# jshilong/GPT4RoI

Hardware: NVIDIA B200
Metric: samples_per_sec_prefill_336px_8roi_128tok_7b (higher is better)
Workload: dtype bf16

## Files before the change

gpt4roi_b200/csrc/attention_tcgen05.cu:

```cuda
#include <stdlib.h>

#include "common.cuh"
#include "ptx.cuh"
#include "act_type.cuh"

namespace G4R_NS {

constexpr int kFaBM = 128;
constexpr int kFaThreads = 256;
constexpr int kAtomBytes = 128 * 128;

struct FaParams {
  __nv_bfloat16* out;
  long long ldo, bso;
  int L, H;
  float scale;
  const int* seqlens;
  float* lse;
};

__device__ __forceinline__ void tmem_st_32x32b_x32(uint32_t taddr, const uint32_t (&r)[32]) {
  asm volatile(
      "tcgen05.st.sync.aligned.32x32b.x32.b32 [%0], "
      "{%1, %2, %3, %4, %5, %6, %7, %8, %9, %10, %11, %12, %13, %14, %15, %16, "
      "%17, %18, %19, %20, %21, %22, %23, %24, %25, %26, %27, %28, %29, %30, %31, %32};"
      ::"r"(taddr), "r"(r[0]), "r"(r[1]), "r"(r[2]), "r"(r[3]), "r"(r[4]), "r"(r[5]), "r"(r[6]), "r"(r[7]),
      "r"(r[8]), "r"(r[9]), "r"(r[10]), "r"(r[11]), "r"(r[12]), "r"(r[13]), "r"(r[14]), "r"(r[15]), "r"(r[16]),
      "r"(r[17]), "r"(r[18]), "r"(r[19]), "r"(r[20]), "r"(r[21]), "r"(r[22]), "r"(r[23]), "r"(r[24]),
      "r"(r[25]), "r"(r[26]), "r"(r[27]), "r"(r[28]), "r"(r[29]), "r"(r[30]), "r"(r[31])
      : "memory");
}
__device__ __forceinline__ void tmem_st_wait() { asm volatile("tcgen05.wait::st.sync.aligned;" ::: "memory"); }

using ptx::make_smem_desc_mn_sw128;

template <int D, int BN, bool CAUSAL>
__global__ void __launch_bounds__(kFaThreads, (BN == 64 ? 2 : 1))
fa_fwd_tcgen05(const __grid_constant__ CUtensorMap tm_q, const __grid_constant__ CUtensorMap tm_k,
               const __grid_constant__ CUtensorMap tm_v, const __grid_constant__ FaParams p) {
  constexpr int kFaBN = BN;
  constexpr int ATOMS = D / 64;
  constexpr int Q_BYTES = ATOMS * kAtomBytes;
  constexpr int KV_ATOM = BN * 128;
  constexpr int TILE_BYTES = ATOMS * KV_ATOM;
  constexpr int P_BYTES = (BN / 64) * kAtomBytes;
  constexpr int TMEM_COLS = (2 * BN + D) <= 256 ? 256 : 512;
  extern __shared__ __align__(1024) uint8_t smem[];
  uint8_t* sQ = smem;
  uint8_t* sK = sQ + Q_BYTES;
  uint8_t* sV = sK + 2 * TILE_BYTES;
  uint8_t* sP = sV + 2 * TILE_BYTES;
// ... 1 lines not shown
  uint64_t* q_full = bars;
  uint64_t* k_full = bars + 1;
  uint64_t* k_empty = bars + 3;
  uint64_t* v_full = bars + 5;
  uint64_t* v_empty = bars + 7;
  uint64_t* s_full = bars + 9;
  uint64_t* s_free = bars + 11;
  uint64_t* p_full = bars + 13;
  uint64_t* pv_done = bars + 14;
  uint32_t* tmem_slot = reinterpret_cast<uint32_t*>(bars + 15);

  const int warp = threadIdx.x >> 5, lane = threadIdx.x & 31;
  const int qb = CAUSAL ? (int)(gridDim.x - 1 - blockIdx.x) : (int)blockIdx.x, h = blockIdx.y, b = blockIdx.z;
  const int q0 = qb * kFaBM;
  const int row_base = b * p.L;
  const int Lk = p.seqlens ? min(max(p.seqlens[b], 1), p.L) : p.L;
  const int nblk = CAUSAL ? min((Lk + kFaBN - 1) / kFaBN, (q0 + kFaBM + kFaBN - 1) / kFaBN) : (Lk + kFaBN - 1) / kFaBN;

  if (warp == 0 && lane == 0) {
    ptx::prefetch_tensormap(&tm_q);
    ptx::prefetch_tensormap(&tm_k);
    ptx::prefetch_tensormap(&tm_v);
  }
  if (warp == 1 && lane == 0) {
    ptx::mbar_init(q_full, 1);
    for (int i = 0; i < 2; i++) {
      ptx::mbar_init(&k_full[i], 1);
      ptx::mbar_init(&k_empty[i], 1);
      ptx::mbar_init(&v_full[i], 1);
      ptx::mbar_init(&v_empty[i], 1);
      ptx::mbar_init(&s_full[i], 1);
      ptx::mbar_init(&s_free[i], 128);
    }
    ptx::mbar_init(p_full, 128);
    ptx::mbar_init(pv_done, 1);
    ptx::fence_barrier_init();
  }
  if (warp == 2) ptx::tmem_alloc(tmem_slot, TMEM_COLS);
  ptx::tcgen05_before_thread_sync();
  __syncthreads();
  ptx::tcgen05_after_thread_sync();
  const uint32_t tmem_base = *tmem_slot;
  const uint32_t tmem_o = tmem_base + 2 * kFaBN;

  if (warp == 0) {
    if (lane == 0) {
      ptx::mbar_arrive_expect_tx(q_full, Q_BYTES);
      for (int a = 0; a < ATOMS; a++)
        ptx::tma_load_2d(sQ + a * kAtomBytes, &tm_q, q_full, h * D + a * 64, row_base + q0);
      for (int j = 0; j < nblk; j++) {
        const int st = j & 1;
        const uint32_t ph = (j >> 1) & 1;
        ptx::mbar_wait(&k_empty[st], ph ^ 1);
        ptx::mbar_arrive_expect_tx(&k_full[st], TILE_BYTES);
        for (int a = 0; a < ATOMS; a++)
          ptx::tma_load_2d(sK + st * TILE_BYTES + a * KV_ATOM, &tm_k, &k_full[st], h * D + a * 64,
                           row_base + j * kFaBN);
        ptx::mbar_wait(&v_empty[st], ph ^ 1);
// ... 54 lines not shown
    constexpr float kTau = 8.0f;
    float m_used = -INFINITY, l_run = 0.f;
    for (int j = 0; j < nblk; j++) {
      const int sb = j & 1;
      ptx::mbar_wait(&s_full[sb], (j >> 1) & 1);
      ptx::tcgen05_after_thread_sync();
      const uint32_t ts = tmem_base + sb * kFaBN + lane_off;
      const int key0 = j * kFaBN;
      const bool need_mask = (key0 + kFaBN > Lk) || (CAUSAL && key0 + kFaBN - 1 > q0);
      uint32_t sv[kFaBN / 32][32];
#pragma unroll
      for (int cc = 0; cc < kFaBN / 32; cc++) ptx::tmem_ld_32x32b_x32(ts + cc * 32, sv[cc]);
      ptx::tmem_ld_wait();
      ptx::tcgen05_before_thread_sync();
      ptx::mbar_arrive(&s_free[sb]);
      float mx = -INFINITY;
#pragma unroll
      for (int cc = 0; cc < kFaBN / 32; cc++) {
#pragma unroll
        for (int i = 0; i < 32; i++) {
          float sc = __uint_as_float(sv[cc][i]);
          if (need_mask) {
            const int key = key0 + cc * 32 + i;
            if (key >= Lk || (CAUSAL && key > qrow)) sc = -INFINITY;
            sv[cc][i] = __float_as_uint(sc);
          }
          mx = fmaxf(mx, sc);
        }
      }
      const float m_new = fmaxf(m_used, mx);
      const bool grow = (m_new - m_used) * c > kTau;
      float alpha = 1.f;
      if (grow) {
        alpha = exp2f((m_used - m_new) * c);
        m_used = m_new;
      }
      const float mc = (m_used == -INFINITY ? 0.f : m_used) * c;
      uint32_t pk[kFaBN / 2];
      float lsum = 0.f;
#pragma unroll
      for (int cc = 0; cc < kFaBN / 32; cc++) {
#pragma unroll
        for (int i = 0; i < 16; i++) {
          const float p0 = exp2f(fmaf(__uint_as_float(sv[cc][2 * i]), c, -mc));
          const float p1 = exp2f(fmaf(__uint_as_float(sv[cc][2 * i + 1]), c, -mc));
          lsum += p0 + p1;
          __nv_bfloat162 hh = __floats2bfloat162_rn(p0, p1);
          pk[cc * 16 + i] = *reinterpret_cast<uint32_t*>(&hh);
        }
      }
      l_run = l_run * alpha + lsum;
      if (j > 0) {
        ptx::mbar_wait(pv_done, (j - 1) & 1);
        ptx::tcgen05_after_thread_sync();
        if (__any_sync(0xffffffffu, grow)) {
#pragma unroll 1
          for (int cc = 0; cc < D / 32; cc++) {
            uint32_t v[32];
            ptx::tmem_ld_32x32b_x32(tmem_o + lane_off + cc * 32, v);
            ptx::tmem_ld_wait();
#pragma unroll
            for (int i = 0; i < 32; i++) v[i] = __float_as_uint(__uint_as_float(v[i]) * alpha);
            tmem_st_32x32b_x32(tmem_o + lane_off + cc * 32, v);
// ... 69 lines not shown
  }
  cuuint64_t dims[2] = {(cuuint64_t)cols, (cuuint64_t)rows};
  cuuint64_t str[1] = {(cuuint64_t)ld * 2};
  cuuint32_t box[2] = {64, (cuuint32_t)box_rows};
  cuuint32_t estr[2] = {1, 1};
  CUresult r = enc(m, CU_TENSOR_MAP_DATA_TYPE_BFLOAT16, 2, const_cast<void*>(base), dims, str, box, estr,
                   CU_TENSOR_MAP_INTERLEAVE_NONE, CU_TENSOR_MAP_SWIZZLE_128B, CU_TENSOR_MAP_L2_PROMOTION_L2_256B,
                   CU_TENSOR_MAP_FLOAT_OOB_FILL_NONE);
  if (r != CUDA_SUCCESS) {
    set_error("attention: cuTensorMapEncodeTiled failed (CUresult %d)", (int)r);
    return G4R_ECUDA;
  }
  return G4R_OK;
}

template <int D, int BN, bool CAUSAL>
static int launch_fa(const CUtensorMap& tq, const CUtensorMap& tk, const CUtensorMap& tv, const FaParams& p, int B,
                     cudaStream_t st) {
  constexpr int smem = (D / 64) * kAtomBytes + 4 * (D / 64) * BN * 128 + (BN / 64) * kAtomBytes + 256;
  static bool set = false;
  auto kern = fa_fwd_tcgen05<D, BN, CAUSAL>;
  if (!set) {
    G4R_CUDA(cudaFuncSetAttribute(kern, cudaFuncAttributeMaxDynamicSharedMemorySize, smem));
    set = true;
  }
  dim3 grid((p.L + kFaBM - 1) / kFaBM, p.H, B);
  kern<<<grid, kFaThreads, smem, st>>>(tq, tk, tv, p);
  G4R_LAUNCH_CHECK("fa_fwd_tcgen05");
  return G4R_OK;
}

}

using namespace G4R_NS;

static int attention_tc_impl(const void* q, const void* k, const void* v, void* out, long long ld,
                             long long bs, long long ldo, long long bso, int B, int H, int L,
                             int head_dim, int causal, float scale, const int* seqlens, float* lse, void* stream) {
  G4R_REQUIRE(q && k && v && out && B > 0 && H > 0 && L > 0, "attention_tc: bad arguments");
  G4R_REQUIRE(head_dim == 64 || head_dim == 128, "attention_tc: head_dim %d (64 or 128)", head_dim);
  G4R_REQUIRE(bs == (long long)L * ld, "attention_tc: q/k/v must be one packed [B*L, width] buffer (bs == L*ld)");
  G4R_REQUIRE(ld % 8 == 0 && ldo % 8 == 0 && bso % 8 == 0, "attention_tc: strides must keep 16-byte alignment");
  G4R_REQUIRE((((uintptr_t)q | (uintptr_t)k | (uintptr_t)v | (uintptr_t)out) & 15) == 0, "attention_tc: misaligned pointers");
  CUtensorMap tq, tk, tv;
  const long long cols = (long long)H * head_dim, rows = (long long)B * L;
  int rc;
  static int bn = 0;
  if (!bn) {
    const char* e = getenv("G4R_ATTN_BN");
    bn = (e && atoi(e) == 128) ? 128 : 64;
  }
  if ((rc = make_tmap_rows(&tq, q, cols, rows, ld, 128))) return rc;
  if ((rc = make_tmap_rows(&tk, k, cols, rows, ld, bn))) return rc;
  if ((rc = make_tmap_rows(&tv, v, cols, rows, ld, bn))) return rc;
  FaParams p{(__nv_bfloat16*)out, ldo, bso, L, H, scale, seqlens, lse};
  cudaStream_t st = (cudaStream_t)stream;
#define G4R_FA(DD, BB) (causal ? launch_fa<DD, BB, true>(tq, tk, tv, p, B, st) : launch_fa<DD, BB, false>(tq, tk, tv, p, B, st))
  if (head_dim == 64) return bn == 128 ? G4R_FA(64, 128) : G4R_FA(64, 64);
  return bn == 128 ? G4R_FA(128, 128) : G4R_FA(128, 64);
#undef G4R_FA
}

extern "C" int g4r_attention_tc_bf16(const void* q, const void* k, const void* v, void* out, long long ld,
                                     long long bs, long long ldo, long long bso, int B, int H, int L,
                                     int head_dim, int causal, float scale, const int* seqlens, void* stream) {
  return attention_tc_impl(q, k, v, out, ld, bs, ldo, bso, B, H, L, head_dim, causal, scale, seqlens, nullptr, stream);
}

#if G4R_BF16_ONLY
extern "C" int g4r_attention_tc_lse_bf16(const void* q, const void* k, const void* v, void* out, long long ld,
                                         long long bs, long long ldo, long long bso, int B, int H, int L,
                                         int head_dim, int causal, float scale, float* lse, void* stream) {
  G4R_REQUIRE(lse, "attention_tc_lse: lse is NULL");
  return attention_tc_impl(q, k, v, out, ld, bs, ldo, bso, B, H, L, head_dim, causal, scale, nullptr, lse, stream);
}
// ... 2 lines not shown
```

gpt4roi_b200/csrc/common.cuh:

```cuda
#pragma once
#include <cuda_bf16.h>
#include <cuda_fp16.h>
#include <cuda_runtime.h>
#include <stdarg.h>
#include <stdint.h>
#include <stdio.h>

#include "../../include/gpt4roi_b200.h"

namespace g4r {

void set_error(const char* fmt, ...);
int cuda_fail(cudaError_t e, const char* what);

#define G4R_REQUIRE(cond, ...)        \
  do {                                \
    if (!(cond)) {                    \
      g4r::set_error(__VA_ARGS__);    \
      return G4R_EINVAL;              \
    }                                 \
  } while (0)

#define G4R_CUDA(call)                                        \
  do {                                                        \
// ... 27 lines not shown
  if (mode == 2) pdl_release();
  pdl_wait();
  if (mode != 2) pdl_release();
}

template <typename... KArgs, typename... Args>
static inline cudaError_t launch_pdl(void (*kern)(KArgs...), dim3 grid, dim3 block, size_t smem, cudaStream_t st,
                                     dim3 cluster, Args... args) {
  cudaLaunchConfig_t cfg = {};
  cfg.gridDim = grid;
  cfg.blockDim = block;
  cfg.dynamicSmemBytes = smem;
  cfg.stream = st;
  cudaLaunchAttribute attr[2];
  int n = 0;
  attr[n].id = cudaLaunchAttributeClusterDimension;
  attr[n].val.clusterDim.x = cluster.x; attr[n].val.clusterDim.y = cluster.y; attr[n].val.clusterDim.z = cluster.z;
  n++;
  if (pdl_mode() != 0) {
    attr[n].id = cudaLaunchAttributeProgrammaticStreamSerialization;
    attr[n].val.programmaticStreamSerializationAllowed = 1;
    n++;
  }
  cfg.attrs = attr;
  cfg.numAttrs = n;
  return cudaLaunchKernelEx(&cfg, kern, static_cast<KArgs>(args)...);
}

template <typename T> __device__ __forceinline__ float to_f32(T v);
template <> __device__ __forceinline__ float to_f32<float>(float v) { return v; }
template <> __device__ __forceinline__ float to_f32<__half>(__half v) { return __half2float(v); }
template <> __device__ __forceinline__ float to_f32<__nv_bfloat16>(__nv_bfloat16 v) { return __bfloat162float(v); }

// ... 39 lines not shown
```

gpt4roi_b200/csrc/elementwise.cu:

```cuda
#include "common.cuh"
#include "act_type.cuh"

namespace G4R_NS {

__device__ __forceinline__ float warp_sum(float v) {
#pragma unroll
  for (int o = 16; o > 0; o >>= 1) v += __shfl_xor_sync(0xffffffffu, v, o);
  return v;
}

__device__ __forceinline__ void unpack8(const uint4& raw, float (&f)[8]) {
  const __nv_bfloat162* h = reinterpret_cast<const __nv_bfloat162*>(&raw);
#pragma unroll
  for (int i = 0; i < 4; i++) {
    const float2 t = __bfloat1622float2(h[i]);
    f[2 * i] = t.x;
    f[2 * i + 1] = t.y;
  }
}
__device__ __forceinline__ uint4 pack8(const float (&f)[8]) {
  uint4 raw;
  __nv_bfloat162* h = reinterpret_cast<__nv_bfloat162*>(&raw);
#pragma unroll
  for (int i = 0; i < 4; i++) h[i] = __floats2bfloat162_rn(f[2 * i], f[2 * i + 1]);
// ... 9 lines not shown
}
template <typename T> __device__ __forceinline__ void store8(T* p, const float (&f)[8]);
template <> __device__ __forceinline__ void store8<__nv_bfloat16>(__nv_bfloat16* p, const float (&f)[8]) {
  *reinterpret_cast<uint4*>(p) = pack8(f);
}
template <> __device__ __forceinline__ void store8<float>(float* p, const float (&f)[8]) {
  reinterpret_cast<float4*>(p)[0] = make_float4(f[0], f[1], f[2], f[3]);
  reinterpret_cast<float4*>(p)[1] = make_float4(f[4], f[5], f[6], f[7]);
}
__device__ __forceinline__ float bf16_round(float x) { return __bfloat162float(__float2bfloat16_rn(x)); }

template <bool RMS, int PER_LANE, typename TI = __nv_bfloat16, typename TO = __nv_bfloat16>
__global__ void __launch_bounds__(256, (sizeof(TI) == 2 && PER_LANE >= 16 ? 2 : 1))
norm_rows_bf16(const TI* __restrict__ x, long long ldx, const __nv_bfloat16* __restrict__ w,
               const __nv_bfloat16* __restrict__ b, TO* __restrict__ out, long long ldo, int M,
               int D, float eps) {
  const int row = blockIdx.x * (blockDim.x >> 5) + (threadIdx.x >> 5);
  if (row >= M) return;
  const int lane = threadIdx.x & 31;
  const int nvec = D >> 3;
  const TI* xr = x + (long long)row * ldx;
  constexpr bool PACKED = sizeof(TI) == 2;
  uint4 raw[PACKED ? PER_LANE : 1];
  float v[PACKED ? 1 : PER_LANE][8];
  float sum = 0.f, sumsq = 0.f;
#pragma unroll
  for (int i = 0; i < PER_LANE; i++) {
    const int vi = lane + (i << 5);
    float t[8];
    if (vi < nvec) {
      if constexpr (PACKED) { raw[i] = *reinterpret_cast<const uint4*>(xr + vi * 8); unpack8(raw[i], t); }
// ... 144 lines not shown
    const int per = (D / 8 + 255) / 256;
#define G4R_NORM_ROW_CASE(PR)                                                                              \
  G4R_CUDA(launch_pdl(norm_row_cta_bf16<RMS, PR>, dim3(M), dim3(256), 0, st, dim3(1, 1, 1),                \
                      (const __nv_bfloat16*)x, ldx, (const __nv_bfloat16*)w, (const __nv_bfloat16*)b,     \
                      (__nv_bfloat16*)out, ldo, D, eps, pdl_mode()))
    if (per <= 1) G4R_NORM_ROW_CASE(1);
    else if (per <= 2) G4R_NORM_ROW_CASE(2);
    else G4R_NORM_ROW_CASE(4);
#undef G4R_NORM_ROW_CASE
    G4R_LAUNCH_CHECK(RMS ? "rmsnorm" : "layernorm");
    return G4R_OK;
  }
  const int per_lane = (D / 8 + 31) / 32;
  const dim3 grid((M + 7) / 8);
#define G4R_NORM_CASE(PL)                                                                              \
  norm_rows_bf16<RMS, PL><<<grid, 256, 0, st>>>((const __nv_bfloat16*)x, ldx, (const __nv_bfloat16*)w,   \
                                                 (const __nv_bfloat16*)b, (__nv_bfloat16*)out, ldo, M, D, eps)
  if (per_lane <= 1) G4R_NORM_CASE(1);
  else if (per_lane <= 2) G4R_NORM_CASE(2);
  else if (per_lane <= 4) G4R_NORM_CASE(4);
  else if (per_lane <= 8) G4R_NORM_CASE(8);
  else if (per_lane <= 16) G4R_NORM_CASE(16);
  else G4R_NORM_CASE(32);
#undef G4R_NORM_CASE
  G4R_LAUNCH_CHECK(RMS ? "rmsnorm" : "layernorm");
  return G4R_OK;
}

template <typename TI, typename TO, bool RMS = false>
static int launch_ln_ex(const void* x, long long ldx, const void* w, const void* b, void* out, long long ldo,
                        int M, int D, float eps, cudaStream_t st) {
  const int per_lane = (D / 8 + 31) / 32;
  const dim3 grid((M + 7) / 8);
#define G4R_LN_CASE(PL)                                                                                   \
  norm_rows_bf16<RMS, PL, TI, TO><<<grid, 256, 0, st>>>((const TI*)x, ldx, (const __nv_bfloat16*)w,        \
                                                        (const __nv_bfloat16*)b, (TO*)out, ldo, M, D, eps)
  if (per_lane <= 1) G4R_LN_CASE(1);
  else if (per_lane <= 2) G4R_LN_CASE(2);
  else if (per_lane <= 4) G4R_LN_CASE(4);
  else if (per_lane <= 8) G4R_LN_CASE(8);
  else if (per_lane <= 16) G4R_LN_CASE(16);
  else G4R_LN_CASE(32);
#undef G4R_LN_CASE
  G4R_LAUNCH_CHECK("layernorm_ex");
  return G4R_OK;
}

__global__ void __launch_bounds__(256)
cast_rows_f32_bf16(const float* __restrict__ x, long long ld, long long bst, __nv_bfloat16* __restrict__ out,
                   int B, int rows_per_batch, int D) {
  const int nvec = D >> 3;
// ... 707 lines not shown
```

gpt4roi_b200/csrc/gemm_tcgen05.cu:

```cuda
#include <stdlib.h>

#include "common.cuh"
#include "ptx.cuh"
#include "act_type.cuh"

namespace G4R_NS {

constexpr int kBlockM = 128;
constexpr int kBlockK = 64;
constexpr int kUmmaK = 16;
constexpr int kGemmThreads = 256;
constexpr int kEpiWarp0 = 4;
constexpr int kSmemBudget = 200 * 1024;

enum { ACT_NONE = 0, ACT_RELU = 1, ACT_QUICK_GELU = 2, ACT_SWIGLU = 3 };

struct GemmParams {
  int M, N, K;
  int num_m_tiles, num_n_tiles, num_k_blocks;
  int k_splits;
  int n_fast;
  void* D;
  long long ldd;
  const void* bias;
// ... 5 lines not shown
  int act;
  int out_f32;
  int atomic;
  int conv;
  int cH, cW, cBH, cBW, tiles_x, tiles_y, cin_blocks, taps;
  int a_rows;
  int levels, lvl_img_stride;
  const __nv_bfloat16* rope_cos;
  const __nv_bfloat16* rope_sin;
  int rope_cols, rope_L, rope_pos0;
  const int* rope_pos_dev;
  int a_mn, b_mn, dw_cin;
  float* gn_stats;
  int gn_group_ch;
  int gn_groups;
};

template <int BLOCK_N>
struct GemmCfg {
  static constexpr int kABytes = kBlockM * kBlockK * 2;
  static constexpr int kBBytes = BLOCK_N * kBlockK * 2;
  static constexpr int kStageBytes = kABytes + kBBytes;
  static constexpr int kStages = kSmemBudget / kStageBytes;
  static constexpr int kAccStages = 2;
  static constexpr int kTmemCols = kAccStages * BLOCK_N;
  static constexpr int kBarBytes = (2 * kStages + 2 * kAccStages) * 8 + 16;
  static constexpr int kSmemBytes = kStages * kStageBytes + kBarBytes + 1024;
};

__device__ __forceinline__ float act_apply(float x, int act) {
// ... 245 lines not shown
    for (int i = 0; i < Cfg::kStages; i++) {
      ptx::mbar_init(&full[i], 1);
      ptx::mbar_init(&empty[i], 1);
    }
    for (int i = 0; i < Cfg::kAccStages; i++) {
      ptx::mbar_init(&tmem_full[i], 1);
      ptx::mbar_init(&tmem_empty[i], 128);
    }
    ptx::fence_barrier_init();
  }
  if (warp == 2) ptx::tmem_alloc(tmem_slot, Cfg::kTmemCols);
  ptx::tcgen05_before_thread_sync();
  __syncthreads();
  ptx::tcgen05_after_thread_sync();
  const uint32_t tmem_base = *tmem_slot;

  const int tiles_mn = p.num_m_tiles * p.num_n_tiles;
  const int total_tiles = tiles_mn * p.k_splits;

  if (warp == 0) {
    if (lane == 0) {
      int stage = 0;
      uint32_t phase = 0;
      for (int t = blockIdx.x; t < total_tiles; t += gridDim.x) {
        const int split = t / tiles_mn;
        const int mn = t % tiles_mn;
        const int n_blk = p.n_fast ? mn % p.num_n_tiles : mn / p.num_m_tiles;
        const int m_blk = p.n_fast ? mn / p.num_n_tiles : mn % p.num_m_tiles;
        const int kb0 = split * p.num_k_blocks;
        int img = 0, y0 = 0, x0 = 0;
        if (CONV) {
          const int tx = m_blk % p.tiles_x;
          const int ty = (m_blk / p.tiles_x) % p.tiles_y;
          img = m_blk / (p.tiles_x * p.tiles_y);
          y0 = ty * p.cBH;
          x0 = tx * p.cBW;
        }
        for (int kb = 0; kb < p.num_k_blocks; kb++) {
          ptx::mbar_wait(&empty[stage], phase ^ 1);
          ptx::mbar_arrive_expect_tx(&full[stage], (uint32_t)(p.a_rows * kBlockK * 2 + Cfg::kBBytes));
          const int kg = kb0 + kb;
          if (CONV) {
            const int tap_all = kg / p.cin_blocks, cc = kg % p.cin_blocks;
            const int lvl = tap_all / p.taps, tap = tap_all % p.taps;
            const int dy = p.taps == 9 ? tap / 3 - 1 : 0, dx = p.taps == 9 ? tap % 3 - 1 : 0;
            ptx::tma_load_4d(smem_a + stage * Cfg::kABytes, &tmap_a, &full[stage], cc * kBlockK, x0 + dx,
                             y0 + dy, img + lvl * p.lvl_img_stride);
          } else if (p.a_mn) {
#pragma unroll
            for (int a = 0; a < kBlockM / 64; a++)
              ptx::tma_load_2d(smem_a + stage * Cfg::kABytes + a * (kBlockK * 128), &tmap_a, &full[stage],
                               m_blk * kBlockM + a * 64, kg * kBlockK);
          } else {
            ptx::tma_load_2d(smem_a + stage * Cfg::kABytes, &tmap_a, &full[stage], kg * kBlockK,
                             m_blk * kBlockM);
          }
          if (!CONV && p.b_mn == 2) {
            const int n0 = n_blk * BLOCK_N, tap = n0 / p.dw_cin, c0 = n0 % p.dw_cin;
#pragma unroll
            for (int a = 0; a < BLOCK_N / 64; a++)
              ptx::tma_load_4d(smem_b + stage * Cfg::kBBytes + a * (kBlockK * 128), &tmap_b, &full[stage],
                               c0 + a * 64, tap % 3, kg * kBlockK, tap / 3);
          } else if (!CONV && p.b_mn) {
#pragma unroll
            for (int a = 0; a < BLOCK_N / 64; a++)
              ptx::tma_load_2d(smem_b + stage * Cfg::kBBytes + a * (kBlockK * 128), &tmap_b, &full[stage],
                               n_blk * BLOCK_N + a * 64, kg * kBlockK);
          } else {
            ptx::tma_load_2d(smem_b + stage * Cfg::kBBytes, &tmap_b, &full[stage], kg * kBlockK, n_blk * BLOCK_N);
          }
          if (++stage == Cfg::kStages) { stage = 0; phase ^= 1; }
        }
      }
    }
  } else if (warp == 1) {
    const uint32_t idesc = ptx::make_idesc_bf16_f32(kBlockM, BLOCK_N) | (p.a_mn ? 1u << 15 : 0u) | (p.b_mn ? 1u << 16 : 0u);
    int stage = 0;
    uint32_t phase = 0;
    int it = 0;
    for (int t = blockIdx.x; t < total_tiles; t += gridDim.x, it++) {
      const int acc = it & 1;
      const uint32_t acc_phase = (it >> 1) & 1;
      ptx::mbar_wait(&tmem_empty[acc], acc_phase ^ 1);
      ptx::tcgen05_after_thread_sync();
      const uint32_t tmem_d = tmem_base + acc * BLOCK_N;
      for (int kb = 0; kb < p.num_k_blocks; kb++) {
        ptx::mbar_wait(&full[stage], phase);
        ptx::tcgen05_after_thread_sync();
// ... 82 lines not shown
      ptx::mbar_init(&full[i], 2);
      ptx::mbar_init(&empty[i], 1);
    }
    for (int i = 0; i < Cfg::kAccStages; i++) {
      ptx::mbar_init(&tmem_full[i], 1);
      ptx::mbar_init(&tmem_empty[i], 256);
    }
    ptx::fence_barrier_init();
  }
  ptx::cluster_sync();
  if (warp == 2) ptx::tmem_alloc_2sm(tmem_slot, Cfg::kTmemCols);
  ptx::tcgen05_before_thread_sync();
  ptx::cluster_sync();
  ptx::tcgen05_after_thread_sync();
  const uint32_t tmem_base = *tmem_slot;

  const int num_m_pairs = (p.num_m_tiles + 1) >> 1;
  const int tiles_mn = num_m_pairs * p.num_n_tiles;
  const int total_tiles = tiles_mn * p.k_splits;
  const int cluster_id = blockIdx.x >> 1, num_clusters = gridDim.x >> 1;

  if (warp == 0) {
    if (lane == 0) {
      int stage = 0;
      uint32_t phase = 0;
      for (int t = cluster_id; t < total_tiles; t += num_clusters) {
        const int split = t / tiles_mn;
        const int mn = t % tiles_mn;
        const int n_blk = p.n_fast ? mn % p.num_n_tiles : mn / num_m_pairs;
        const int m_blk = (p.n_fast ? mn / p.num_n_tiles : mn % num_m_pairs) * 2 + (int)rank;
        const int kb0 = split * p.num_k_blocks;
        int img = 0, y0 = 0, x0 = 0;
        if (CONV) {
          const int tx = m_blk % p.tiles_x;
          const int ty = (m_blk / p.tiles_x) % p.tiles_y;
          img = m_blk / (p.tiles_x * p.tiles_y);
          y0 = ty * p.cBH;
          x0 = tx * p.cBW;
        }
        for (int kb = 0; kb < p.num_k_blocks; kb++) {
          ptx::mbar_wait(&empty[stage], phase ^ 1);
          const int kg = kb0 + kb;
          if (CONV) {
            const int tap_all = kg / p.cin_blocks, cc = kg % p.cin_blocks;
            const int lvl = tap_all / p.taps, tap = tap_all % p.taps;
            const int dy = p.taps == 9 ? tap / 3 - 1 : 0, dx = p.taps == 9 ? tap % 3 - 1 : 0;
            const int im = img < p.lvl_img_stride ? img + lvl * p.lvl_img_stride : p.lvl_img_stride * p.levels;
            ptx::tma_load_4d_2sm(smem_a + stage * Cfg::kABytes, &tmap_a, &full[stage], cc * kBlockK, x0 + dx,
                                 y0 + dy, im);
          } else if (p.a_mn) {
#pragma unroll
            for (int a = 0; a < kBlockM / 64; a++)
              ptx::tma_load_2d_2sm(smem_a + stage * Cfg::kABytes + a * (kBlockK * 128), &tmap_a, &full[stage],
                                   m_blk * kBlockM + a * 64, kg * kBlockK);
          } else {
            ptx::tma_load_2d_2sm(smem_a + stage * Cfg::kABytes, &tmap_a, &full[stage], kg * kBlockK,
                                 m_blk * kBlockM);
          }
          const int nb0 = n_blk * BLOCK_N + (int)rank * (BLOCK_N / 2);
          if (!CONV && p.b_mn == 2) {
            const int tap = nb0 / p.dw_cin, c0 = nb0 % p.dw_cin;
#pragma unroll
            for (int a = 0; a < BLOCK_N / 2 / 64; a++)
              ptx::tma_load_4d_2sm(smem_b + stage * Cfg::kBBytes + a * (kBlockK * 128), &tmap_b, &full[stage],
                                   c0 + a * 64, tap % 3, kg * kBlockK, tap / 3);
          } else if (!CONV && p.b_mn) {
#pragma unroll
            for (int a = 0; a < BLOCK_N / 2 / 64; a++)
              ptx::tma_load_2d_2sm(smem_b + stage * Cfg::kBBytes + a * (kBlockK * 128), &tmap_b, &full[stage],
                                   nb0 + a * 64, kg * kBlockK);
          } else {
            ptx::tma_load_2d_2sm(smem_b + stage * Cfg::kBBytes, &tmap_b, &full[stage], kg * kBlockK, nb0);
          }
          if (leader) {
            ptx::mbar_arrive_expect_tx(&full[stage], 2u * (uint32_t)(p.a_rows * kBlockK * 2 + Cfg::kBBytes));
          } else {
            ptx::mbar_arrive_cluster(&full[stage], 0);
          }
          if (++stage == Cfg::kStages) { stage = 0; phase ^= 1; }
        }
      }
    }
  } else if (warp == 1 && leader) {
    const uint32_t idesc = ptx::make_idesc_bf16_f32(2 * kBlockM, BLOCK_N) | (p.a_mn ? 1u << 15 : 0u) | (p.b_mn ? 1u << 16 : 0u);
    int stage = 0;
    uint32_t phase = 0;
    int it = 0;
    for (int t = cluster_id; t < total_tiles; t += num_clusters, it++) {
      const int acc = it & 1;
      const uint32_t acc_phase = (it >> 1) & 1;
      ptx::mbar_wait(&tmem_empty[acc], acc_phase ^ 1);
      ptx::tcgen05_after_thread_sync();
      const uint32_t tmem_d = tmem_base + acc * BLOCK_N;
      for (int kb = 0; kb < p.num_k_blocks; kb++) {
        ptx::mbar_wait(&full[stage], phase);
        ptx::tcgen05_after_thread_sync();
// ... 73 lines not shown
  }
  return G4R_OK;
}

template <int BLOCK_N, bool CONV>
static int launch_gemm(const CUtensorMap& ta, const CUtensorMap& tb, const GemmParams& p, cudaStream_t st) {
  using Cfg = GemmCfg<BLOCK_N>;
  static bool attr_set = false;
  auto kern = gemm_bf16_tcgen05<BLOCK_N, CONV>;
  if (!attr_set) {
    G4R_CUDA(cudaFuncSetAttribute(kern, cudaFuncAttributeMaxDynamicSharedMemorySize, Cfg::kSmemBytes));
    attr_set = true;
  }
  const int total = p.num_m_tiles * p.num_n_tiles * p.k_splits;
  const int grid = total < sm_budget() ? total : sm_budget();
  kern<<<grid, kGemmThreads, Cfg::kSmemBytes, st>>>(ta, tb, p);
  G4R_LAUNCH_CHECK("gemm_bf16_tcgen05");
  return G4R_OK;
}

template <bool CONV>
static int launch_gemm_2sm(const CUtensorMap& ta, const CUtensorMap& tb, const GemmParams& p, cudaStream_t st) {
  using Cfg = Gemm2Cfg;
  static bool attr_set = false;
  auto kern = gemm_bf16_tcgen05_2sm<CONV>;
  if (!attr_set) {
    G4R_CUDA(cudaFuncSetAttribute(kern, cudaFuncAttributeMaxDynamicSharedMemorySize, Cfg::kSmemBytes));
    attr_set = true;
  }
  const int pairs = ((p.num_m_tiles + 1) / 2) * p.num_n_tiles * p.k_splits;
  const int max_clusters = sm_budget() / 2;
  const int clusters = pairs < max_clusters ? pairs : max_clusters;
  kern<<<2 * clusters, kGemmThreads, Cfg::kSmemBytes, st>>>(ta, tb, p);
  G4R_LAUNCH_CHECK("gemm_bf16_tcgen05_2sm");
  return G4R_OK;
}

static bool use_2sm(int N, int m_tiles, int k_splits, bool conv) {
  static int env = -1;
  if (env < 0) {
    const char* e = getenv("G4R_GEMM_2SM");
    env = !e ? 1 : (e[0] == '0' ? 0 : (e[0] == '2' ? 2 : 1));
  }
  if (env == 0 || (env == 2 && !conv) || N <= 128 || m_tiles < 2) return false;
  const long pairs = (long)((m_tiles + 1) / 2) * ((N + 255) / 256) * k_splits;
  return pairs >= num_sms() / 2;
}

static int pick_block_n(int N, int m_tiles, int k_splits) {
  if (N <= 128) return 128;
  const long t256 = (long)m_tiles * ((N + 255) / 256) * k_splits;
  if (t256 >= num_sms()) return 256;
  return 128;
}

}

using namespace G4R_NS;

extern "C" int g4r_gemm_bf16(const void* A, long long lda, const void* B, long long ldb, void* D,
                             long long ldd, int M, int N, int K, const void* bias, int bias_f32,
                             const void* residual, long long ldr, int act, int out_f32, int k_splits,
                             void* stream);
extern "C" int g4r_gemm_bf16_ex(const void* A, long long lda, const void* B, long long ldb, void* D,
                                long long ldd, int M, int N, int K, const void* bias, int bias_f32,
                                const void* residual, long long ldr, int residual_f32, int bias_round_bf16,
                                int act, int out_f32, int k_splits, void* stream);
extern "C" int g4r_gemm_bf16(const void* A, long long lda, const void* B, long long ldb, void* D,
// ... 141 lines not shown
  }
  GemmParams p{};
  p.M = M; p.N = N; p.K = K;
  p.num_m_tiles = (M + kBlockM - 1) / kBlockM;
  const int kb_total = (K + kBlockK - 1) / kBlockK;
  G4R_REQUIRE(kb_total % k_splits == 0, "K blocks (%d) not divisible by k_splits (%d)", kb_total, k_splits);
  p.k_splits = k_splits;
  p.num_k_blocks = kb_total / k_splits;
  p.D = D; p.ldd = ldd; p.bias = bias; p.bias_f32 = bias_f32;
  p.residual = (const __nv_bfloat16*)residual; p.ldr = ldr; p.residual_f32 = residual_f32;
  p.round_branch = bias_round_bf16;
  p.rope_cos = (const __nv_bfloat16*)rope_cos; p.rope_sin = (const __nv_bfloat16*)rope_sin;
  p.rope_cols = rope_cols; p.rope_L = rope_L; p.rope_pos0 = rope_pos0; p.rope_pos_dev = rope_pos_dev;
  p.act = act; p.out_f32 = out_f32; p.atomic = k_splits > 1;
  p.conv = 0; p.a_rows = kBlockM;
  const bool two = use_2sm(N, p.num_m_tiles, k_splits, false);
  const int bn = two ? 256 : pick_block_n(N, p.num_m_tiles, k_splits);
  p.num_n_tiles = (N + bn - 1) / bn;
  CUtensorMap ta, tb;
  {
    cuuint64_t dims[2] = {(cuuint64_t)K, (cuuint64_t)M};
    cuuint64_t str[1] = {(cuuint64_t)lda * 2};
    cuuint32_t box[2] = {kBlockK, kBlockM};
    int rc = make_tmap(&ta, A, 2, dims, str, box);
    if (rc) return rc;
  }
  {
    cuuint64_t dims[2] = {(cuuint64_t)K, (cuuint64_t)N};
    cuuint64_t str[1] = {(cuuint64_t)ldb * 2};
    cuuint32_t box[2] = {kBlockK, (cuuint32_t)(two ? bn / 2 : bn)};
    int rc = make_tmap(&tb, B, 2, dims, str, box);
// ... 80 lines not shown
```

gpt4roi_b200/engine.py:

```python
import math

import torch

from . import dense, kernels
from .roi_align import roi_align_mlvl
from .splice import splice_region_tokens

BF16 = torch.bfloat16


class EngineConfig:
    def __init__(self, image_size=336, patch_size=14, vit_hidden=1024, vit_heads=16, vit_layers=24,
                 vit_mlp=4096, vit_eps=1e-5, select_layer=-2, num_levels=4,
                 hidden=4096, n_heads=32, n_layers=32, mlp=11008, vocab=32006, rms_eps=1e-6,
                 rope_theta=10000.0, roi_out=14, roi_sampling=2, spi_dim=1024, gn_groups=64,
                 im_patch_token=32001, bbox_token=32002, im_start_token=32004, im_end_token=32005,
                 llama_stream=None, dtype='bf16'):
        import os
        if llama_stream is None:
            llama_stream = os.environ.get('G4R_LLAMA_STREAM', 'bf16')
        if llama_stream not in ('fp32', 'bf16'):
            raise ValueError('llama_stream must be fp32 or bf16 (bf16 = the 16-bit storage type)')
        if dtype in (torch.bfloat16, torch.float16):
            dtype = 'bf16' if dtype == torch.bfloat16 else 'fp16'
# ... 231 lines not shown
        if bboxes is None or len(bboxes) == 0:
            return None
        counts = [0 if b is None else int(b.shape[0]) for b in bboxes]
        K = sum(counts)
        offs = torch.tensor([0] + list(torch.tensor(counts).cumsum(0).tolist()), dtype=torch.int32).to(self.dev)
        if K > 0:
            boxes = torch.cat([b.to(self.dev, torch.float32) for b in bboxes if b is not None and b.shape[0]], 0).contiguous()
            bidx = torch.cat([torch.full((n,), float(i)) for i, n in enumerate(counts)]).to(self.dev)
        else:
            boxes = torch.zeros((0, 4), dtype=torch.float32, device=self.dev)
            bidx = torch.zeros((0,), dtype=torch.float32, device=self.dev)
        return dict(K=K, boxes=boxes, bidx=bidx, offs=offs)

    def forward_device(self, input_ids, images, plan, validate=True, last_only=False, seqlens=None, cache=None,
                       hidden_taps=None, want='logits', stage_taps=None):
        c = self.cfg
        B, L = input_ids.shape
        if images is None:
            embeds = splice_region_tokens(input_ids, self.embed, None, None, 0, c.im_patch_token, c.im_start_token,
                                          c.im_end_token, c.bbox_token, validate=False)
            if cache is not None:
                cache.length = L
            return self.llama(embeds, B, L, last_only=last_only, seqlens=seqlens, cache=cache,
                              hidden_taps=hidden_taps, want=want)
        taps = self.vit(images)
        feat = kernels.cast_tokens_f32_bf16(taps[c.select_index], dtype=self.dt)
        img_rows = dense.linear(feat, self.proj_w, self.proj_b).view(B, c.num_patches, c.hidden)
        region = None
        if plan is not None:
            if plan['K'] > 0:
# ... 257 lines not shown
```

Measured before the change: 68.48.

## Enable PDL across attention, norm and GEMM kernels; add GEMM M-tail 1SM heuristic

Switches the attention, norm and GEMM launches to programmatic dependent launch and turns PDL on for the whole device forward pass, so each kernel's setup overlaps the tail of the previous one. GEMM producers prefetch weight (B) tiles before the dependency wait. A heuristic now picks 1-SM GEMM tiles over 2-SM clusters when the M tile count is odd. The change also adds an env-gated polynomial exp2 split in attention and a 4-way max reduction. The risks are PDL ordering bugs, such as reading seqlens or activations before the wait, and a hand-tuned heuristic constant.

New measurement: 69.62, median of 6. 1.7% higher.

```diff
diff --git a/gpt4roi_b200/csrc/attention_tcgen05.cu b/gpt4roi_b200/csrc/attention_tcgen05.cu
--- a/gpt4roi_b200/csrc/attention_tcgen05.cu
+++ b/gpt4roi_b200/csrc/attention_tcgen05.cu
@@ -1,4 +1,5 @@
 #include <stdlib.h>
+#include <string.h>
 
 #include "common.cuh"
 #include "ptx.cuh"
@@ -17,6 +18,7 @@
   float scale;
   const int* seqlens;
   float* lse;
+  int pdl;
 };
 
 __device__ __forceinline__ void tmem_st_32x32b_x32(uint32_t taddr, const uint32_t (&r)[32]) {
@@ -34,7 +36,17 @@
 
 using ptx::make_smem_desc_mn_sw128;
 
-template <int D, int BN, bool CAUSAL>
+__device__ __forceinline__ float exp2_fma(float x) {
+  const float xc = fmaxf(x, -125.f);
+  const float t = __fadd_rn(xc, 12582912.f);
+  const float f = __fsub_rn(xc, __fsub_rn(t, 12582912.f));
+  const float p = fmaf(fmaf(fmaf(0.05517132f, f, 0.24261054f), f, 0.69326097f), f, 0.99992812f);
+  const float r = __int_as_float(__float_as_int(p) + (__float_as_int(t) << 23));
+  return x < -125.f ? 0.f : r;
+}
+constexpr int kExpFmaOf8 = 2;
+
+template <int D, int BN, bool CAUSAL, bool EXP_SPLIT>
 __global__ void __launch_bounds__(kFaThreads, (BN == 64 ? 2 : 1))
 fa_fwd_tcgen05(const __grid_constant__ CUtensorMap tm_q, const __grid_constant__ CUtensorMap tm_k,
                const __grid_constant__ CUtensorMap tm_v, const __grid_constant__ FaParams p) {
@@ -66,8 +78,6 @@
   const int qb = CAUSAL ? (int)(gridDim.x - 1 - blockIdx.x) : (int)blockIdx.x, h = blockIdx.y, b = blockIdx.z;
   const int q0 = qb * kFaBM;
   const int row_base = b * p.L;
-  const int Lk = p.seqlens ? min(max(p.seqlens[b], 1), p.L) : p.L;
-  const int nblk = CAUSAL ? min((Lk + kFaBN - 1) / kFaBN, (q0 + kFaBM + kFaBN - 1) / kFaBN) : (Lk + kFaBN - 1) / kFaBN;
 
   if (warp == 0 && lane == 0) {
     ptx::prefetch_tensormap(&tm_q);
@@ -94,6 +104,9 @@
   ptx::tcgen05_after_thread_sync();
   const uint32_t tmem_base = *tmem_slot;
   const uint32_t tmem_o = tmem_base + 2 * kFaBN;
+  pdl_sync(p.pdl);
+  const int Lk = p.seqlens ? min(max(p.seqlens[b], 1), p.L) : p.L;
+  const int nblk = CAUSAL ? min((Lk + kFaBN - 1) / kFaBN, (q0 + kFaBM + kFaBN - 1) / kFaBN) : (Lk + kFaBN - 1) / kFaBN;
 
   if (warp == 0) {
     if (lane == 0) {
@@ -178,7 +191,7 @@
       ptx::tmem_ld_wait();
       ptx::tcgen05_before_thread_sync();
       ptx::mbar_arrive(&s_free[sb]);
-      float mx = -INFINITY;
+      float mx4[4] = {-INFINITY, -INFINITY, -INFINITY, -INFINITY};
 #pragma unroll
       for (int cc = 0; cc < kFaBN / 32; cc++) {
 #pragma unroll
@@ -189,9 +202,10 @@
             if (key >= Lk || (CAUSAL && key > qrow)) sc = -INFINITY;
             sv[cc][i] = __float_as_uint(sc);
           }
-          mx = fmaxf(mx, sc);
-        }
-      }
+          mx4[i & 3] = fmaxf(mx4[i & 3], sc);
+        }
+      }
+      const float mx = fmaxf(fmaxf(mx4[0], mx4[1]), fmaxf(mx4[2], mx4[3]));
       const float m_new = fmaxf(m_used, mx);
       const bool grow = (m_new - m_used) * c > kTau;
       float alpha = 1.f;
@@ -202,15 +216,35 @@
       const float mc = (m_used == -INFINITY ? 0.f : m_used) * c;
       uint32_t pk[kFaBN / 2];
       float lsum = 0.f;
-#pragma unroll
-      for (int cc = 0; cc < kFaBN / 32; cc++) {
-#pragma unroll
-        for (int i = 0; i < 16; i++) {
-          const float p0 = exp2f(fmaf(__uint_as_float(sv[cc][2 * i]), c, -mc));
-          const float p1 = exp2f(fmaf(__uint_as_float(sv[cc][2 * i + 1]), c, -mc));
-          lsum += p0 + p1;
-          __nv_bfloat162 hh = __floats2bfloat162_rn(p0, p1);
-          pk[cc * 16 + i] = *reinterpret_cast<uint32_t*>(&hh);
+      if constexpr (EXP_SPLIT) {
+        float ls[8] = {0.f, 0.f, 0.f, 0.f, 0.f, 0.f, 0.f, 0.f};
+#pragma unroll
+        for (int cc = 0; cc < kFaBN / 32; cc++) {
+#pragma unroll
+          for (int i = 0; i < 16; i++) {
+            float pp[2];
+#pragma unroll
+            for (int e = 0; e < 2; e++) {
+              const float x = fmaf(__uint_as_float(sv[cc][2 * i + e]), c, -mc);
+              pp[e] = ((2 * i + e) & 7) < 8 - kExpFmaOf8 ? exp2f(x) : exp2_fma(x);
+            }
+            ls[i & 7] += pp[0] + pp[1];
+            __nv_bfloat162 hh = __floats2bfloat162_rn(pp[0], pp[1]);
+            pk[cc * 16 + i] = *reinterpret_cast<uint32_t*>(&hh);
+          }
+        }
+        lsum = ((ls[0] + ls[1]) + (ls[2] + ls[3])) + ((ls[4] + ls[5]) + (ls[6] + ls[7]));
+      } else {
+#pragma unroll
+        for (int cc = 0; cc < kFaBN / 32; cc++) {
+#pragma unroll
+          for (int i = 0; i < 16; i++) {
+            const float p0 = exp2f(fmaf(__uint_as_float(sv[cc][2 * i]), c, -mc));
+            const float p1 = exp2f(fmaf(__uint_as_float(sv[cc][2 * i + 1]), c, -mc));
+            lsum += p0 + p1;
+            __nv_bfloat162 hh = __floats2bfloat162_rn(p0, p1);
+            pk[cc * 16 + i] = *reinterpret_cast<uint32_t*>(&hh);
+          }
         }
       }
       l_run = l_run * alpha + lsum;
@@ -310,19 +344,18 @@
   return G4R_OK;
 }
 
-template <int D, int BN, bool CAUSAL>
+template <int D, int BN, bool CAUSAL, bool EXP_SPLIT>
 static int launch_fa(const CUtensorMap& tq, const CUtensorMap& tk, const CUtensorMap& tv, const FaParams& p, int B,
                      cudaStream_t st) {
   constexpr int smem = (D / 64) * kAtomBytes + 4 * (D / 64) * BN * 128 + (BN / 64) * kAtomBytes + 256;
   static bool set = false;
-  auto kern = fa_fwd_tcgen05<D, BN, CAUSAL>;
+  auto kern = fa_fwd_tcgen05<D, BN, CAUSAL, EXP_SPLIT>;
   if (!set) {
     G4R_CUDA(cudaFuncSetAttribute(kern, cudaFuncAttributeMaxDynamicSharedMemorySize, smem));
     set = true;
   }
   dim3 grid((p.L + kFaBM - 1) / kFaBM, p.H, B);
-  kern<<<grid, kFaThreads, smem, st>>>(tq, tk, tv, p);
-  G4R_LAUNCH_CHECK("fa_fwd_tcgen05");
+  G4R_CUDA(launch_pdl(kern, grid, dim3(kFaThreads), smem, st, dim3(1, 1, 1), tq, tk, tv, p));
   return G4R_OK;
 }
 
@@ -349,12 +382,19 @@
   if ((rc = make_tmap_rows(&tq, q, cols, rows, ld, 128))) return rc;
   if ((rc = make_tmap_rows(&tk, k, cols, rows, ld, bn))) return rc;
   if ((rc = make_tmap_rows(&tv, v, cols, rows, ld, bn))) return rc;
-  FaParams p{(__nv_bfloat16*)out, ldo, bso, L, H, scale, seqlens, lse};
+  static int split = -1;
+  if (split < 0) {
+    const char* e = getenv("G4R_ATTN_EXP");
+    split = (e && strcmp(e, "fma") == 0) ? 1 : 0;
+  }
+  FaParams p{(__nv_bfloat16*)out, ldo, bso, L, H, scale, seqlens, lse, pdl_mode()};
   cudaStream_t st = (cudaStream_t)stream;
-#define G4R_FA(DD, BB) (causal ? launch_fa<DD, BB, true>(tq, tk, tv, p, B, st) : launch_fa<DD, BB, false>(tq, tk, tv, p, B, st))
+#define G4R_FA2(DD, BB, CC) (split ? launch_fa<DD, BB, CC, true>(tq, tk, tv, p, B, st) : launch_fa<DD, BB, CC, false>(tq, tk, tv, p, B, st))
+#define G4R_FA(DD, BB) (causal ? G4R_FA2(DD, BB, true) : G4R_FA2(DD, BB, false))
   if (head_dim == 64) return bn == 128 ? G4R_FA(64, 128) : G4R_FA(64, 64);
   return bn == 128 ? G4R_FA(128, 128) : G4R_FA(128, 64);
 #undef G4R_FA
+#undef G4R_FA2
 }
 
 extern "C" int g4r_attention_tc_bf16(const void* q, const void* k, const void* v, void* out, long long ld,
diff --git a/gpt4roi_b200/csrc/common.cuh b/gpt4roi_b200/csrc/common.cuh
--- a/gpt4roi_b200/csrc/common.cuh
+++ b/gpt4roi_b200/csrc/common.cuh
@@ -65,9 +65,11 @@
   cfg.stream = st;
   cudaLaunchAttribute attr[2];
   int n = 0;
-  attr[n].id = cudaLaunchAttributeClusterDimension;
-  attr[n].val.clusterDim.x = cluster.x; attr[n].val.clusterDim.y = cluster.y; attr[n].val.clusterDim.z = cluster.z;
-  n++;
+  if (cluster.x != 0) {
+    attr[n].id = cudaLaunchAttributeClusterDimension;
+    attr[n].val.clusterDim.x = cluster.x; attr[n].val.clusterDim.y = cluster.y; attr[n].val.clusterDim.z = cluster.z;
+    n++;
+  }
   if (pdl_mode() != 0) {
     attr[n].id = cudaLaunchAttributeProgrammaticStreamSerialization;
     attr[n].val.programmaticStreamSerializationAllowed = 1;
diff --git a/gpt4roi_b200/csrc/elementwise.cu b/gpt4roi_b200/csrc/elementwise.cu
--- a/gpt4roi_b200/csrc/elementwise.cu
+++ b/gpt4roi_b200/csrc/elementwise.cu
@@ -47,7 +47,8 @@
 __global__ void __launch_bounds__(256, (sizeof(TI) == 2 && PER_LANE >= 16 ? 2 : 1))
 norm_rows_bf16(const TI* __restrict__ x, long long ldx, const __nv_bfloat16* __restrict__ w,
                const __nv_bfloat16* __restrict__ b, TO* __restrict__ out, long long ldo, int M,
-               int D, float eps) {
+               int D, float eps, int pdl) {
+  pdl_sync(pdl);
   const int row = blockIdx.x * (blockDim.x >> 5) + (threadIdx.x >> 5);
   if (row >= M) return;
   const int lane = threadIdx.x & 31;
@@ -222,8 +223,9 @@
   const int per_lane = (D / 8 + 31) / 32;
   const dim3 grid((M + 7) / 8);
 #define G4R_NORM_CASE(PL)                                                                              \
-  norm_rows_bf16<RMS, PL><<<grid, 256, 0, st>>>((const __nv_bfloat16*)x, ldx, (const __nv_bfloat16*)w,   \
-                                                 (const __nv_bfloat16*)b, (__nv_bfloat16*)out, ldo, M, D, eps)
+  G4R_CUDA(launch_pdl(norm_rows_bf16<RMS, PL>, grid, dim3(256), 0, st, dim3(1, 1, 1), (const __nv_bfloat16*)x, ldx, \
+                      (const __nv_bfloat16*)w, (const __nv_bfloat16*)b, (__nv_bfloat16*)out, ldo, M, D, eps,        \
+                      pdl_mode()))
   if (per_lane <= 1) G4R_NORM_CASE(1);
   else if (per_lane <= 2) G4R_NORM_CASE(2);
   else if (per_lane <= 4) G4R_NORM_CASE(4);
@@ -241,8 +243,8 @@
   const int per_lane = (D / 8 + 31) / 32;
   const dim3 grid((M + 7) / 8);
 #define G4R_LN_CASE(PL)                                                                                   \
-  norm_rows_bf16<RMS, PL, TI, TO><<<grid, 256, 0, st>>>((const TI*)x, ldx, (const __nv_bfloat16*)w,        \
-                                                        (const __nv_bfloat16*)b, (TO*)out, ldo, M, D, eps)
+  G4R_CUDA(launch_pdl(norm_rows_bf16<RMS, PL, TI, TO>, grid, dim3(256), 0, st, dim3(1, 1, 1), (const TI*)x, ldx, \
+                      (const __nv_bfloat16*)w, (const __nv_bfloat16*)b, (TO*)out, ldo, M, D, eps, pdl_mode()))
   if (per_lane <= 1) G4R_LN_CASE(1);
   else if (per_lane <= 2) G4R_LN_CASE(2);
   else if (per_lane <= 4) G4R_LN_CASE(4);
diff --git a/gpt4roi_b200/csrc/gemm_tcgen05.cu b/gpt4roi_b200/csrc/gemm_tcgen05.cu
--- a/gpt4roi_b200/csrc/gemm_tcgen05.cu
+++ b/gpt4roi_b200/csrc/gemm_tcgen05.cu
@@ -43,6 +43,7 @@
   float* gn_stats;
   int gn_group_ch;
   int gn_groups;
+  int pdl;
 };
 
 template <int BLOCK_N>
@@ -318,6 +319,7 @@
   __syncthreads();
   ptx::tcgen05_after_thread_sync();
   const uint32_t tmem_base = *tmem_slot;
+  if (warp != 0) pdl_sync(p.pdl);
 
   const int tiles_mn = p.num_m_tiles * p.num_n_tiles;
   const int total_tiles = tiles_mn * p.k_splits;
@@ -326,6 +328,34 @@
     if (lane == 0) {
       int stage = 0;
       uint32_t phase = 0;
+      auto load_b = [&](int st, int n_blk, int kg) {
+        if (!CONV && p.b_mn == 2) {
+          const int n0 = n_blk * BLOCK_N, tap = n0 / p.dw_cin, c0 = n0 % p.dw_cin;
+#pragma unroll
+          for (int a = 0; a < BLOCK_N / 64; a++)
+            ptx::tma_load_4d(smem_b + st * Cfg::kBBytes + a * (kBlockK * 128), &tmap_b, &full[st],
+                             c0 + a * 64, tap % 3, kg * kBlockK, tap / 3);
+        } else if (!CONV && p.b_mn) {
+#pragma unroll
+          for (int a = 0; a < BLOCK_N / 64; a++)
+            ptx::tma_load_2d(smem_b + st * Cfg::kBBytes + a * (kBlockK * 128), &tmap_b, &full[st],
+                             n_blk * BLOCK_N + a * 64, kg * kBlockK);
+        } else {
+          ptx::tma_load_2d(smem_b + st * Cfg::kBBytes, &tmap_b, &full[st], kg * kBlockK, n_blk * BLOCK_N);
+        }
+      };
+      int pre = 0;
+      if (p.pdl && (int)blockIdx.x < total_tiles) {
+        const int mn = (int)blockIdx.x % tiles_mn;
+        const int n_blk = p.n_fast ? mn % p.num_n_tiles : mn / p.num_m_tiles;
+        const int kb0 = ((int)blockIdx.x / tiles_mn) * p.num_k_blocks;
+        pre = p.num_k_blocks < Cfg::kStages ? p.num_k_blocks : Cfg::kStages;
+        for (int kb = 0; kb < pre; kb++) {
+          ptx::mbar_arrive_expect_tx(&full[kb], (uint32_t)(p.a_rows * kBlockK * 2 + Cfg::kBBytes));
+          load_b(kb, n_blk, kb0 + kb);
+        }
+      }
+      pdl_sync(p.pdl);
       for (int t = blockIdx.x; t < total_tiles; t += gridDim.x) {
         const int split = t / tiles_mn;
         const int mn = t % tiles_mn;
@@ -341,8 +371,11 @@
           x0 = tx * p.cBW;
         }
         for (int kb = 0; kb < p.num_k_blocks; kb++) {
-          ptx::mbar_wait(&empty[stage], phase ^ 1);
-          ptx::mbar_arrive_expect_tx(&full[stage], (uint32_t)(p.a_rows * kBlockK * 2 + Cfg::kBBytes));
+          const bool prefetched = t == (int)blockIdx.x && kb < pre;
+          if (!prefetched) {
+            ptx::mbar_wait(&empty[stage], phase ^ 1);
+            ptx::mbar_arrive_expect_tx(&full[stage], (uint32_t)(p.a_rows * kBlockK * 2 + Cfg::kBBytes));
+          }
           const int kg = kb0 + kb;
           if (CONV) {
             const int tap_all = kg / p.cin_blocks, cc = kg % p.cin_blocks;
@@ -359,23 +392,12 @@
             ptx::tma_load_2d(smem_a + stage * Cfg::kABytes, &tmap_a, &full[stage], kg * kBlockK,
                              m_blk * kBlockM);
           }
-          if (!CONV && p.b_mn == 2) {
-            const int n0 = n_blk * BLOCK_N, tap = n0 / p.dw_cin, c0 = n0 % p.dw_cin;
-#pragma unroll
-            for (int a = 0; a < BLOCK_N / 64; a++)
-              ptx::tma_load_4d(smem_b + stage * Cfg::kBBytes + a * (kBlockK * 128), &tmap_b, &full[stage],
-                               c0 + a * 64, tap % 3, kg * kBlockK, tap / 3);
-          } else if (!CONV && p.b_mn) {
-#pragma unroll
-            for (int a = 0; a < BLOCK_N / 64; a++)
-              ptx::tma_load_2d(smem_b + stage * Cfg::kBBytes + a * (kBlockK * 128), &tmap_b, &full[stage],
-                               n_blk * BLOCK_N + a * 64, kg * kBlockK);
-          } else {
-            ptx::tma_load_2d(smem_b + stage * Cfg::kBBytes, &tmap_b, &full[stage], kg * kBlockK, n_blk * BLOCK_N);
-          }
+          if (!prefetched) load_b(stage, n_blk, kg);
           if (++stage == Cfg::kStages) { stage = 0; phase ^= 1; }
         }
       }
+    } else {
+      pdl_sync(p.pdl);
     }
   } else if (warp == 1) {
     const uint32_t idesc = ptx::make_idesc_bf16_f32(kBlockM, BLOCK_N) | (p.a_mn ? 1u << 15 : 0u) | (p.b_mn ? 1u << 16 : 0u);
@@ -488,6 +510,7 @@
   ptx::cluster_sync();
   ptx::tcgen05_after_thread_sync();
   const uint32_t tmem_base = *tmem_slot;
+  if (warp != 0) pdl_sync(p.pdl);
 
   const int num_m_pairs = (p.num_m_tiles + 1) >> 1;
   const int tiles_mn = num_m_pairs * p.num_n_tiles;
@@ -498,6 +521,42 @@
     if (lane == 0) {
       int stage = 0;
       uint32_t phase = 0;
+      auto load_b = [&](int st, int n_blk, int kg) {
+        const int nb0 = n_blk * BLOCK_N + (int)rank * (BLOCK_N / 2);
+        if (!CONV && p.b_mn == 2) {
+          const int tap = nb0 / p.dw_cin, c0 = nb0 % p.dw_cin;
+#pragma unroll
+          for (int a = 0; a < BLOCK_N / 2 / 64; a++)
+            ptx::tma_load_4d_2sm(smem_b + st * Cfg::kBBytes + a * (kBlockK * 128), &tmap_b, &full[st],
+                                 c0 + a * 64, tap % 3, kg * kBlockK, tap / 3);
+        } else if (!CONV && p.b_mn) {
+#pragma unroll
+          for (int a = 0; a < BLOCK_N / 2 / 64; a++)
+            ptx::tma_load_2d_2sm(smem_b + st * Cfg::kBBytes + a * (kBlockK * 128), &tmap_b, &full[st],
+                                 nb0 + a * 64, kg * kBlockK);
+        } else {
+          ptx::tma_load_2d_2sm(smem_b + st * Cfg::kBBytes, &tmap_b, &full[st], kg * kBlockK, nb0);
+        }
+      };
+      auto arrive_full = [&](int st) {
+        if (leader) {
+          ptx::mbar_arrive_expect_tx(&full[st], 2u * (uint32_t)(p.a_rows * kBlockK * 2 + Cfg::kBBytes));
+        } else {
+          ptx::mbar_arrive_cluster(&full[st], 0);
+        }
+      };
+      int pre = 0;
+      if (p.pdl && cluster_id < total_tiles) {
+        const int mn = cluster_id % tiles_mn;
+        const int n_blk = p.n_fast ? mn % p.num_n_tiles : mn / num_m_pairs;
+        const int kb0 = (cluster_id / tiles_mn) * p.num_k_blocks;
+        pre = p.num_k_blocks < Cfg::kStages ? p.num_k_blocks : Cfg::kStages;
+        for (int kb = 0; kb < pre; kb++) {
+          load_b(kb, n_blk, kb0 + kb);
+          arrive_full(kb);
+        }
+      }
+      pdl_sync(p.pdl);
       for (int t = cluster_id; t < total_tiles; t += num_clusters) {
         const int split = t / tiles_mn;
         const int mn = t % tiles_mn;
@@ -513,7 +572,8 @@
           x0 = tx * p.cBW;
         }
         for (int kb = 0; kb < p.num_k_blocks; kb++) {
-          ptx::mbar_wait(&empty[stage], phase ^ 1);
+          const bool prefetched = t == cluster_id && kb < pre;
+          if (!prefetched) ptx::mbar_wait(&empty[stage], phase ^ 1);
           const int kg = kb0 + kb;
           if (CONV) {
             const int tap_all = kg / p.cin_blocks, cc = kg % p.cin_blocks;
@@ -531,29 +591,15 @@
             ptx::tma_load_2d_2sm(smem_a + stage * Cfg::kABytes, &tmap_a, &full[stage], kg * kBlockK,
                                  m_blk * kBlockM);
           }
-          const int nb0 = n_blk * BLOCK_N + (int)rank * (BLOCK_N / 2);
-          if (!CONV && p.b_mn == 2) {
-            const int tap = nb0 / p.dw_cin, c0 = nb0 % p.dw_cin;
-#pragma unroll
-            for (int a = 0; a < BLOCK_N / 2 / 64; a++)
-              ptx::tma_load_4d_2sm(smem_b + stage * Cfg::kBBytes + a * (kBlockK * 128), &tmap_b, &full[stage],
-                                   c0 + a * 64, tap % 3, kg * kBlockK, tap / 3);
-          } else if (!CONV && p.b_mn) {
-#pragma unroll
-            for (int a = 0; a < BLOCK_N / 2 / 64; a++)
-              ptx::tma_load_2d_2sm(smem_b + stage * Cfg::kBBytes + a * (kBlockK * 128), &tmap_b, &full[stage],
-                                   nb0 + a * 64, kg * kBlockK);
-          } else {
-            ptx::tma_load_2d_2sm(smem_b + stage * Cfg::kBBytes, &tmap_b, &full[stage], kg * kBlockK, nb0);
-          }
-          if (leader) {
-            ptx::mbar_arrive_expect_tx(&full[stage], 2u * (uint32_t)(p.a_rows * kBlockK * 2 + Cfg::kBBytes));
-          } else {
-            ptx::mbar_arrive_cluster(&full[stage], 0);
+          if (!prefetched) {
+            load_b(stage, n_blk, kg);
+            arrive_full(stage);
           }
           if (++stage == Cfg::kStages) { stage = 0; phase ^= 1; }
         }
       }
+    } else {
+      pdl_sync(p.pdl);
     }
   } else if (warp == 1 && leader) {
     const uint32_t idesc = ptx::make_idesc_bf16_f32(2 * kBlockM, BLOCK_N) | (p.a_mn ? 1u << 15 : 0u) | (p.b_mn ? 1u << 16 : 0u);
@@ -657,8 +703,9 @@
   }
   const int total = p.num_m_tiles * p.num_n_tiles * p.k_splits;
   const int grid = total < sm_budget() ? total : sm_budget();
-  kern<<<grid, kGemmThreads, Cfg::kSmemBytes, st>>>(ta, tb, p);
-  G4R_LAUNCH_CHECK("gemm_bf16_tcgen05");
+  GemmParams q = p;
+  q.pdl = pdl_mode();
+  G4R_CUDA(launch_pdl(kern, dim3(grid), dim3(kGemmThreads), Cfg::kSmemBytes, st, dim3(1, 1, 1), ta, tb, q));
   return G4R_OK;
 }
 
@@ -674,8 +721,9 @@
   const int pairs = ((p.num_m_tiles + 1) / 2) * p.num_n_tiles * p.k_splits;
   const int max_clusters = sm_budget() / 2;
   const int clusters = pairs < max_clusters ? pairs : max_clusters;
-  kern<<<2 * clusters, kGemmThreads, Cfg::kSmemBytes, st>>>(ta, tb, p);
-  G4R_LAUNCH_CHECK("gemm_bf16_tcgen05_2sm");
+  GemmParams q = p;
+  q.pdl = pdl_mode();
+  G4R_CUDA(launch_pdl(kern, dim3(2 * clusters), dim3(kGemmThreads), Cfg::kSmemBytes, st, dim3(0, 0, 0), ta, tb, q));
   return G4R_OK;
 }
 
@@ -695,6 +743,19 @@
   const long t256 = (long)m_tiles * ((N + 255) / 256) * k_splits;
   if (t256 >= num_sms()) return 256;
   return 128;
+}
+
+static bool mtail_prefers_1sm(int N, int m_tiles, int k_splits) {
+  static int env = -1;
+  if (env < 0) { const char* e = getenv("G4R_GEMM_MTAIL"); env = (e && e[0] == '0') ? 0 : 1; }
+  if (!env || m_tiles % 2 == 0) return false;
+  const long clusters = sm_budget() / 2;
+  const long pair_tiles = (long)((m_tiles + 1) / 2) * ((N + 255) / 256) * k_splits;
+  const long rounds_2sm = (pair_tiles + clusters - 1) / clusters;
+  const int bn = pick_block_n(N, m_tiles, k_splits);
+  const long tiles = (long)m_tiles * ((N + bn - 1) / bn) * k_splits;
+  const long rounds_1sm = (tiles + sm_budget() - 1) / sm_budget();
+  return (double)rounds_1sm * (bn == 256 ? 1.0 : 0.5) / 0.93 < (double)rounds_2sm;
 }
 
 }
@@ -866,7 +927,7 @@
   p.rope_cols = rope_cols; p.rope_L = rope_L; p.rope_pos0 = rope_pos0; p.rope_pos_dev = rope_pos_dev;
   p.act = act; p.out_f32 = out_f32; p.atomic = k_splits > 1;
   p.conv = 0; p.a_rows = kBlockM;
-  const bool two = use_2sm(N, p.num_m_tiles, k_splits, false);
+  const bool two = use_2sm(N, p.num_m_tiles, k_splits, false) && !mtail_prefers_1sm(N, p.num_m_tiles, k_splits);
   const int bn = two ? 256 : pick_block_n(N, p.num_m_tiles, k_splits);
   p.num_n_tiles = (N + bn - 1) / bn;
   CUtensorMap ta, tb;
diff --git a/gpt4roi_b200/engine.py b/gpt4roi_b200/engine.py
--- a/gpt4roi_b200/engine.py
+++ b/gpt4roi_b200/engine.py
@@ -269,6 +269,16 @@
 
     def forward_device(self, input_ids, images, plan, validate=True, last_only=False, seqlens=None, cache=None,
                        hidden_taps=None, want='logits', stage_taps=None):
+        from . import lib
+        prev = lib.set_pdl(True)
+        try:
+            return self._forward_device(input_ids, images, plan, validate, last_only, seqlens, cache, hidden_taps,
+                                        want, stage_taps)
+        finally:
+            lib.set_pdl(prev)
+
+    def _forward_device(self, input_ids, images, plan, validate, last_only, seqlens, cache, hidden_taps, want,
+                        stage_taps):
         c = self.cfg
         B, L = input_ids.shape
         if images is None:
```
